# akashsengupta1997/STRAPS-3DHumanShapePose

Measured on AMD Instinct MI355X. Metric: bodies/sec, higher is better.
Workload: dtype fp32 (encoder convolutions as exact bf16x3 operand splits (six bf16 products per term); in-step SMPL blend contraction and skinning as 3-product fp16 splits (fp16x3_lbs: 22-bit operands); fp32 accumulate throughout)

## Files before the change

straps-3dhumanshapepose_amd/csrc/conv_wgrad.hip:

```cpp
#include "conv_wgrad_kernels.h"

namespace {

constexpr int F_TAP_F32 = STRAPS_WG_FAMILY_TAP_F32, F_HALO_F32 = STRAPS_WG_FAMILY_HALO_F32, F_TAP_X3 = STRAPS_WG_FAMILY_TAP_X3,
              F_HALO_X3 = STRAPS_WG_FAMILY_HALO_X3, F_TAP_X3F = STRAPS_WG_FAMILY_TAP_X3F;
constexpr int HALO_NG = 2;

inline int splits_for(int target, int tiles, long long max_s) {
    long long s = (target + tiles - 1) / tiles;
    if (s > max_s) s = max_s;
    return s < 1 ? 1 : (int)s;
}

bool halo_plan(int family, int cp, int batch, int h, int w, int cin, int cout, int kh, int kw, int stride, int pad, WgradPlan* pl) {
    if (!(kh == 3 && kw == 3 && stride == 1 && pad == 1)) return false;
    if (w < 8 || (w & (w - 1)) != 0) return false;
    const int cw = w < 32 ? w : 32, rpc = cp / cw;
    if (h % rpc != 0) return false;
    int lg = 0;
    while ((1 << lg) < cw) ++lg;
    WgradHaloGeom& g = pl->halo;
    g = {h, w, cin, cout, cw, lg, rpc, w / cw, h / rpc, batch * (h / rpc) * (w / cw), 0, cin / 64};
    const int tiles = (cout / 64) * (cin / 64);
    const int s = splits_for(WGRAD_CUS, tiles, (g.nchunks + 3) / 4);
    g.chunks_per_split = (g.nchunks + s - 1) / s;
    const int lds = family == F_HALO_F32 ? HALO_NG * 2 * W3PX * 64 * 4 : 2 * 3 * (cp + (cp == 32 ? 128 : 136)) * 64 * 2;
    pl->q = {family, 64, 64, cp, tiles, (g.nchunks + g.chunks_per_split - 1) / g.chunks_per_split, g.chunks_per_split, g.nchunks, 9, lds, 0};
    return true;
}

inline int tap_lds(int family, int bco, int bci) { return 2 * 32 * (bco + bci) * (family == F_TAP_F32 ? 4 : 3 * 2); }

void tap_plan(int family, int bco, int bci, int target, long long max_s, WgradPlan* pl) {
    WgradTapGeom& g = pl->tap;
    g.ct = g.Cout / bco; g.it = g.Cin / bci;
    const int taps = g.R * g.S, tiles = taps * g.ct * g.it, splits = splits_for(target, tiles, max_s);
    g.rows_per_split = (int)((((long long)g.M + splits - 1) / splits + 31) / 32 * 32);
    pl->q = {family, bco, bci, 0, tiles, splits, g.rows_per_split, g.M, taps, tap_lds(family, bco, bci), 0};
}

inline bool wgrad_big_tile(const WgradTapGeom& g) { return g.Cin % 128 == 0 && g.Cout % 128 == 0 && g.R * g.S == 1 && g.M >= 8192; }

void tap_f32_plan(WgradPlan* pl) {
    const bool big = wgrad_big_tile(pl->tap);
    tap_plan(F_TAP_F32, big ? 128 : 64, big ? 128 : 64, (big ? 2 : 6) * WGRAD_CUS, ((long long)pl->tap.M + 127) / 128, pl);
}

void tap_x3_block(const WgradTapGeom& g, int* bco, int* bci) {
    const int cin = g.Cin, cout = g.Cout;
    *bco = *bci = wgrad_big_tile(g) ? 128 : 64;
    if (g.R * g.S == 1) {
        if (g.M >= 32768 && cout % 256 == 0 && cin % 128 == 0) { *bco = 256; *bci = 128; }
        else if (g.M <= 8192 && cout % 128 == 0 && cin % 128 == 0) {
            if (g.stride == 1 && cout > cin) { *bco = 64; *bci = 128; }
            else { *bco = 128; *bci = 64; }
        }
    } else if (cout % 256 == 0 && cin % 128 == 0) { *bco = 256; *bci = 128; }
    else if (cout % 128 == 0 && cin % 64 == 0) { *bco = 128; *bci = 64; }
}

void tap_x3_plan(int bco, int bci, WgradPlan* pl) {
    const long long max_s = ((long long)pl->tap.M + 127) / 128;
    if (bco == bci) {
        tap_plan(F_TAP_X3, bco, bci, (bco == 128 ? 1 : 6) * WGRAD_CUS, max_s, pl);
        return;
    }
    WgradPlan f32 = *pl;
    tap_f32_plan(&f32);
    const int per_cu = (160 * 1024) / tap_lds(F_TAP_X3, bco, bci);
    tap_plan(F_TAP_X3, bco, bci, WGRAD_CUS * (per_cu < 1 ? 1 : per_cu), max_s < f32.q.splits ? max_s : f32.q.splits, pl);
}

void tap_x3f_block(int cin, int cout, int* bco, int* bci) {
    if (cout % 256 == 0 && cin == 64) { *bco = 256; *bci = 64; }
    else if (cin % 256 == 0 && cout == 64) { *bco = 64; *bci = 256; }
    else if (cout % 256 == 0 && cin % 128 == 0 && cout >= cin) { *bco = 256; *bci = 128; }
    else if (cin % 256 == 0 && cout % 128 == 0) { *bco = 128; *bci = 256; }
    else if (cout % 128 == 0 && cin % 128 == 0) { *bco = 128; *bci = 128; }
    else { *bco = 64; *bci = 64; }
}

inline bool reads_planes(const WgradPlan& pl) { return pl.q.family == F_TAP_X3 || pl.q.family == F_HALO_X3; }

}

int straps_internal_wgrad_plan(const char* who, int form, int batch, int h, int w, int cin, int cout, int kh, int kw, int stride, int pad, WgradPlan* pl) {
    *pl = WgradPlan{};
    const bool planes = form == STRAPS_WG_ROUTE_PLANES, x3f = form == STRAPS_WG_ROUTE_F32_1X1;
    STRAPS_REQUIRE(cin % 64 == 0 && cout % 64 == 0, "%s: need cin%%64==0 and cout%%64==0 (cin=%d cout=%d)", who, cin, cout);
    STRAPS_REQUIRE(!x3f || (kh == 1 && kw == 1 && pad == 0 && stride >= 1), "%s: 1x1 filters without padding only", who);
    WgradTapGeom& g = pl->tap;
    g = {batch, h, w, cin, cout, kh, kw, stride, pad, (h + 2 * pad - kh) / stride + 1, (w + 2 * pad - kw) / stride + 1};
    if (!x3f && halo_plan(planes ? F_HALO_X3 : F_HALO_F32, 32, batch, h, w, cin, cout, kh, kw, stride, pad, pl)) {
        WgradPlan p64 = *pl;
        if (planes && halo_plan(F_HALO_X3, 64, batch, h, w, cin, cout, kh, kw, stride, pad, &p64) && p64.q.splits <= pl->q.splits) *pl = p64;
    } else {
        const long long M = (long long)batch * g.Ho * g.Wo;
        STRAPS_REQUIRE(M < (1LL << 31) && (!x3f || M > 0), "%s: problem too large (or empty)", who);
        g.M = (int)M;
        int bco, bci;
        if (x3f) {
            tap_x3f_block(cin, cout, &bco, &bci);
            tap_plan(F_TAP_X3F, bco, bci, (bco == 64 && bci == 64 ? 2 : 1) * WGRAD_CUS, (M + 63) / 64, pl);
        } else if (planes && (kh * kw > 1 || (cin >= 128 && cout >= 128))) {
            tap_x3_block(g, &bco, &bci);
            tap_x3_plan(bco, bci, pl);
        } else {
            tap_f32_plan(pl);
        }
    }
#ifdef STRAPS_TOOLS
    if (pl->q.family == F_TAP_X3) {
        if (const int v = STRAPS_TOOL_ENV_INT("STRAPS_WGRAD_TILE", 0)) {
            const int o = v / 1000, i = v % 1000, sq = wgrad_big_tile(pl->tap) ? 128 : 64;
            const bool ok = (o == 64 || o == 128 || o == 256) && (i == 64 || i == 128 || i == 256) && !(o == 256 && i == 256) && cout % o == 0 && cin % i == 0 &&
                            !(o == 128 && i == 128 && sq != 128);
            tap_x3_plan(ok ? o : sq, ok ? i : sq, pl);
        }
    }
    static const int abl = STRAPS_TOOL_ENV_INT("STRAPS_WGRAD3_ABL", 0);
    if (pl->q.family == F_HALO_X3 && pl->q.chunk_px == 64) pl->abl = abl;
#endif
    pl->q.part_bytes = (int64_t)pl->q.splits * cout * pl->q.taps * cin * (int64_t)sizeof(float);
    return STRAPS_OK;
}

int straps_internal_wgrad_reduce(const float* part, float* dw_oihw, int splits, int cout, int cin, int taps, int accumulate, hipStream_t st) {
    const long long n = (long long)cout * taps * cin;
    hipLaunchKernelGGL(wgrad_reduce_kernel, dim3((unsigned)(n / 256)), dim3(256), 0, st, part, dw_oihw, splits, cout, cin, taps, accumulate);
    STRAPS_CHECK_LAUNCH("wgrad_reduce_kernel");
    return STRAPS_OK;
}

extern "C" int straps_conv_wgrad_plan(int route, int batch, int h, int w, int cin, int cout, int kh, int kw, int stride, int pad, straps_wgrad_plan_t* out) {
    STRAPS_REQUIRE(out && route >= STRAPS_WG_ROUTE_F32 && route <= STRAPS_WG_ROUTE_F32_1X1, "straps_conv_wgrad_plan: null pointer or unknown route %d", route);
    WgradPlan pl;
    const int rc = straps_internal_wgrad_plan("straps_conv_wgrad_plan", route, batch, h, w, cin, cout, kh, kw, stride, pad, &pl);
    if (rc == STRAPS_OK) *out = pl.q;
    return rc;
}

extern "C" size_t straps_conv_wgrad_workspace_bytes(int batch, int h, int w, int cin, int cout, int kh, int kw, int stride, int pad) {
    WgradPlan pl;
    const int rc = straps_internal_wgrad_plan("straps_conv_wgrad_workspace_bytes", STRAPS_WG_ROUTE_F32, batch, h, w, cin, cout, kh, kw, stride, pad, &pl);
    return rc == STRAPS_OK ? (size_t)pl.q.part_bytes : 0;
}

extern "C" int straps_conv_wgrad_x3_on_planes(int batch, int h, int w, int cin, int cout, int kh, int kw, int stride, int pad) {
    WgradPlan pl;
    return straps_internal_wgrad_plan("straps_conv_wgrad_x3_on_planes", STRAPS_WG_ROUTE_PLANES, batch, h, w, cin, cout, kh, kw, stride, pad, &pl) == STRAPS_OK && reads_planes(pl);
}

namespace {

constexpr int wkey(int family, int chunk_px, int bco, int bci) { return (family << 24) | (chunk_px << 18) | (bco << 9) | bci; }

int wgrad_launch(const WgradPlan& pl, const float* x, const float* dy, const u16* x3, long long xps, const u16* dy3, long long dps, float* dw_oihw,
                 void* workspace, int accumulate, void* stream) {
    const straps_wgrad_plan_t& q = pl.q;
    float* part = (float*)workspace;
    hipStream_t st = (hipStream_t)stream;
    const dim3 grid(q.tiles, q.splits);
    const size_t lds = (size_t)q.lds_bytes;
    WgradP tf{x, dy, part, pl.tap};
    Wgrad3P hf{x, dy, part, pl.halo};
    WgradXP tx{x3, dy3, xps, dps, part, pl.tap};
    Wgrad3XP hx{x3, dy3, xps, dps, part, pl.halo, (long long)pl.tap.B * pl.tap.H * pl.tap.W};
#define WGRAD_LAUNCH(KERN, THREADS, P)                                       \
    do {                                                                     \
        if (lds >= 64 * 1024) STRAPS_RAISE_LDS((KERN), lds, #KERN);          \
        hipLaunchKernelGGL((KERN), grid, dim3(THREADS), lds, st, P);         \
        STRAPS_CHECK_LAUNCH(#KERN);                                          \
    } while (0)
    switch (wkey(q.family, q.chunk_px, q.bco, q.bci)) {
    case wkey(F_TAP_F32, 0, 64, 64): WGRAD_LAUNCH((conv_wgrad_kernel<64, 64>), 256, tf); break;
    case wkey(F_TAP_F32, 0, 128, 128): WGRAD_LAUNCH((conv_wgrad_kernel<128, 128>), 256, tf); break;
    case wkey(F_HALO_F32, 32, 64, 64): WGRAD_LAUNCH((conv_wgrad3x3_kernel<HALO_NG>), 256 * HALO_NG, hf); break;
    case wkey(F_HALO_X3, 32, 64, 64): WGRAD_LAUNCH((conv_wgrad3x3_x3_kernel<HALO_NG, 32>), 256 * HALO_NG, hx); break;
    case wkey(F_HALO_X3, 64, 64, 64):
#ifdef STRAPS_TOOLS
        if (pl.abl) {
            auto kern = pl.abl == 1 ? conv_wgrad3x3_x3_kernel<HALO_NG, 64, 1> : pl.abl == 2 ? conv_wgrad3x3_x3_kernel<HALO_NG, 64, 2>
                      : pl.abl == 3 ? conv_wgrad3x3_x3_kernel<HALO_NG, 64, 3> : pl.abl == 4 ? conv_wgrad3x3_x3_kernel<HALO_NG, 64, 4> : conv_wgrad3x3_x3_kernel<HALO_NG, 64, 5>;
            (void)hipFuncSetAttribute((const void*)kern, hipFuncAttributeMaxDynamicSharedMemorySize, (int)lds);
            hipLaunchKernelGGL(kern, grid, dim3(256 * HALO_NG), lds, st, hx);
            STRAPS_CHECK_LAUNCH("conv_wgrad3x3_x3_kernel (ablation)");
            return STRAPS_OK;
        }
#endif
        WGRAD_LAUNCH((conv_wgrad3x3_x3_kernel<HALO_NG, 64>), 256 * HALO_NG, hx);
        break;
    case wkey(F_TAP_X3, 0, 64, 64): WGRAD_LAUNCH((conv_wgrad_x3_kernel<64, 64>), 256, tx); break;
    case wkey(F_TAP_X3, 0, 128, 128): WGRAD_LAUNCH((conv_wgrad_x3_kernel<128, 128>), 256, tx); break;
    case wkey(F_TAP_X3, 0, 256, 128): WGRAD_LAUNCH((conv_wgrad_x3_kernel<256, 128>), 256, tx); break;
    case wkey(F_TAP_X3, 0, 128, 64): WGRAD_LAUNCH((conv_wgrad_x3_kernel<128, 64>), 256, tx); break;
    case wkey(F_TAP_X3, 0, 64, 128): WGRAD_LAUNCH((conv_wgrad_x3_kernel<64, 128>), 256, tx); break;
#ifdef STRAPS_TOOLS
    case wkey(F_TAP_X3, 0, 256, 64): WGRAD_LAUNCH((conv_wgrad_x3_kernel<256, 64>), 256, tx); break;
    case wkey(F_TAP_X3, 0, 64, 256): WGRAD_LAUNCH((conv_wgrad_x3_kernel<64, 256>), 256, tx); break;
    case wkey(F_TAP_X3, 0, 128, 256): WGRAD_LAUNCH((conv_wgrad_x3_kernel<128, 256>), 256, tx); break;
#endif
    default: STRAPS_REQUIRE(false, "conv weight gradient: no kernel for family %d, block %d x %d", q.family, q.bco, q.bci);
    }
#undef WGRAD_LAUNCH
    return straps_internal_wgrad_reduce(part, dw_oihw, q.splits, pl.tap.Cout, pl.tap.Cin, q.taps, accumulate, st);
}

}

extern "C" int straps_conv_wgrad_x3(const float* x, const float* dy, const unsigned short* x3, long long x_plane_stride, const unsigned short* dy3,
                                    long long dy_plane_stride, float* dw_oihw, void* workspace, int batch, int h, int w, int cin, int cout, int kh,
                                    int kw, int stride, int pad, int accumulate, void* stream) {
    STRAPS_REQUIRE(dw_oihw && workspace, "straps_conv_wgrad_x3: null pointer");
    WgradPlan pl;
    const int rc = straps_internal_wgrad_plan("straps_conv_wgrad_x3", (x3 && dy3) ? STRAPS_WG_ROUTE_PLANES : STRAPS_WG_ROUTE_F32, batch, h, w, cin, cout, kh, kw, stride, pad, &pl);
    if (rc != STRAPS_OK) return rc;
    if (reads_planes(pl)) {
        STRAPS_REQUIRE(x_plane_stride % 8 == 0 && dy_plane_stride % 8 == 0, "straps_conv_wgrad_x3: plane strides must be multiples of 8 elements");
        const size_t adv = straps_conv_wgrad_workspace_bytes(batch, h, w, cin, cout, kh, kw, stride, pad);
        STRAPS_REQUIRE((size_t)pl.q.part_bytes <= adv, "straps_conv_wgrad_x3: the plan's partials (%lld bytes) exceed the advertised workspace (%zu)", (long long)pl.q.part_bytes, adv);
    } else {
        STRAPS_REQUIRE(x && dy, "straps_conv_wgrad_x3: this shape runs on the fp32 tensors, which are NULL (see straps_conv_wgrad_x3_on_planes)");
    }
    return wgrad_launch(pl, x, dy, x3, x_plane_stride, dy3, dy_plane_stride, dw_oihw, workspace, accumulate, stream);
}

extern "C" int straps_conv_wgrad(const float* x, const float* dy, float* dw_oihw, void* workspace, int batch, int h, int w, int cin,
                                 int cout, int kh, int kw, int stride, int pad, int accumulate, void* stream) {
    STRAPS_REQUIRE(x && dy && dw_oihw && workspace, "straps_conv_wgrad: null pointer");
    return straps_conv_wgrad_x3(x, dy, nullptr, 0, nullptr, 0, dw_oihw, workspace, batch, h, w, cin, cout, kh, kw, stride, pad, accumulate, stream);
}
```

straps-3dhumanshapepose_amd/csrc/conv_wgrad_kernels.h:

```cpp
#pragma once
#include "common.h"
#include "conv_wgrad_plan.h"

namespace {

struct WgradP {
    const float* x;
    const float* dy;
    float* part;
    WgradTapGeom g;
};

__device__ __attribute__((aligned(16))) float k_zero16w[4] = {0.f, 0.f, 0.f, 0.f};

template <int BCO, int BCI>
__global__ __launch_bounds__(256) void conv_wgrad_kernel(WgradP p) {
    constexpr int STG = 32 * (BCO + BCI);
    constexpr int LPD = BCO / 4, PWD = 64 / LPD, RDD = 8 / PWD;
    constexpr int LPX = BCI / 4, PWX = 64 / LPX, RDX = 8 / PWX;
    constexpr int MI = BCO / 64, NI = BCI / 64;
    extern __shared__ __attribute__((aligned(16))) float smem[];
    const int tid = threadIdx.x, lane = tid & 63, wave = tid >> 6;
    const int wave_u = __builtin_amdgcn_readfirstlane(wave);
    const int wm = wave >> 1, wn = wave & 1;
// ... 503 lines not shown
#pragma unroll
        for (int q = 0; q < DR; ++q) {
            if (NG > 1 && (q & 1) != grp) continue;
#pragma unroll
            for (int pl = 0; pl < 3; ++pl)
                __builtin_amdgcn_global_load_lds((const __attribute__((address_space(1))) void*)(dbase + d_off[q] + pl * p.dps),
                                                 (__attribute__((address_space(3))) void*)(D + (pl * DPX + 32 * q + 8 * wave_u) * 64), 16, 0, 0);
        }
#pragma unroll
        for (int q = 0; q < XR; ++q) {
            if (q * 32 + 8 * wave_u >= npatch || q * 32 + 8 * wave_u >= XPX) break;
            if (NG > 1 && ((q + DR) & 1) != grp) continue;
            const int hi = ho0 + x_pr[q], wi = wo0 + x_pc[q];
            const bool ok = (unsigned)hi < (unsigned)p.g.H && (unsigned)wi < (unsigned)p.g.W;
            const u16* src = ok ? xsrc + (x_pr[q] * p.g.W + x_pc[q]) * 32 + x_g[q] : zsrc;
            const long long ps = ok ? p.xps : 0;
#pragma unroll
            for (int pl = 0; pl < 3; ++pl)
                __builtin_amdgcn_global_load_lds((const __attribute__((address_space(1))) void*)(src + pl * ps),
                                                 (__attribute__((address_space(3))) void*)(X + (pl * XPX + 32 * q + 8 * wave_u) * 64), 16, 0, 0);
        }
    };

    const int t = lane & 15, ch16 = (lane >> 4) & 1, kh = lane >> 5;
    auto row_off = [&](int slot_px, int c4) {
        const int g = (c4 >> 3) ^ (((slot_px >> 1) & 1) << 2);
        return slot_px * 64 + g * 8 + (c4 & 4);
    };
    int d_fo[KSG][2], x_fo[KSG][2];
#pragma unroll
    for (int ks = 0; ks < KSG; ++ks)
#pragma unroll
        for (int r = 0; r < 2; ++r) {
            const int px = (grp + NG * ks) * 16 + kh * 8 + r * 4 + (t >> 2);
            d_fo[ks][r] = row_off(px, wm * 32 + ch16 * 16 + (t & 3) * 4);
            x_fo[ks][r] = (px >> p.g.cw_log2) * pw + (px & (p.g.cw - 1));
        }
    const int x_c4 = wn * 32 + ch16 * 16 + (t & 3) * 4;

    f32x16 acc[9];
#pragma unroll
    for (int tp = 0; tp < 9; ++tp)
#pragma unroll
        for (int q = 0; q < 16; ++q) acc[tp][q] = 0.f;
    if (cbeg < cend) dma_chunk(cbeg, 0);
    constexpr int TA[6] = {1, 0, 2, 0, 1, 0};
    constexpr int TB[6] = {1, 2, 0, 1, 0, 0};
    for (int c = cbeg; c < cend; ++c) {
        const int stage = (c - cbeg) & 1;
        asm volatile("s_waitcnt vmcnt(0)" ::: "memory");
        __builtin_amdgcn_s_barrier();
        asm volatile("" ::: "memory");
        if (c + 1 < cend && !(ABL & 1)) dma_chunk(c + 1, stage ^ 1);
        const u16* D = smem + ((ABL & 1) ? 0 : stage) * STAGE;
        const u16* X = D + 3 * DPX * 64;
        __builtin_amdgcn_s_setprio(1);
#pragma unroll
        for (int ks = 0; ks < KSG; ++ks) {
            bf16x8w a[3];
#pragma unroll
            for (int pl = 0; pl < 3; ++pl) a[pl] = tr_frag(D + pl * DPX * 64 + d_fo[ks][0], D + pl * DPX * 64 + d_fo[ks][1]);
#pragma unroll
            for (int tp0 = 0; tp0 < 9; tp0 += W3X_TG) {
                bf16x8w b[W3X_TG][3];
#pragma unroll
                for (int u = 0; u < W3X_TG; ++u) {
                    const int tp = tp0 + u;
                    if (tp >= 9) break;
                    const int sh = (ABL & 4) ? 0 : (tp / 3) * pw + (tp % 3);
                    const int o0 = row_off(x_fo[ks][0] + sh, x_c4), o1 = row_off(x_fo[ks][1] + sh, x_c4);
#pragma unroll
                    for (int pl = 0; pl < 3; ++pl) b[u][pl] = tr_frag(X + pl * XPX * 64 + o0, X + pl * XPX * 64 + o1);
                }
                if (ABL & 2) {
#pragma unroll
                    for (int u = 0; u < W3X_TG; ++u)
                        if (tp0 + u < 9)
#pragma unroll
                            for (int pl = 0; pl < 3; ++pl) acc[0][pl] += (float)b[u][pl][0] + (float)a[pl][1];
                    continue;
                }
#pragma unroll
                for (int e = 0; e < 6; ++e)
#pragma unroll
                    for (int u = 0; u < W3X_TG; ++u)
                        if (tp0 + u < 9) acc[tp0 + u] = __builtin_amdgcn_mfma_f32_32x32x16_bf16(a[TA[e]], b[u][TB[e]], acc[tp0 + u], 0, 0, 0);
            }
        }
        __builtin_amdgcn_s_setprio(0);
    }
    if constexpr (NG > 1) {
        float* R = smem_f + ((wave * 3) * 16) * 64 + lane;
#pragma unroll
        for (int rd = 0; rd < 3; ++rd) {
            __syncthreads();
            if (grp == 1) {
#pragma unroll
                for (int tp = 0; tp < 3; ++tp)
#pragma unroll
                    for (int q = 0; q < 16; ++q) R[(tp * 16 + q) * 64] = acc[rd * 3 + tp][q];
            }
            __syncthreads();
            if (grp == 0) {
#pragma unroll
                for (int tp = 0; tp < 3; ++tp)
#pragma unroll
                    for (int q = 0; q < 16; ++q) acc[rd * 3 + tp][q] += R[(tp * 16 + q) * 64];
            }
        }
        if (grp != 0) return;
    }
    const int i = lane & 31;
    float* o = p.part + (long long)blockIdx.y * p.g.Cout * 9 * p.g.Cin;
#pragma unroll
    for (int tp = 0; tp < 9; ++tp)
#pragma unroll
        for (int q = 0; q < 16; ++q) {
            const int co = co0 + wm * 32 + mfma_row(q, lane);
            o[((long long)co * 9 + tp) * p.g.Cin + ci0 + wn * 32 + i] = acc[tp][q];
        }
}

__global__ __launch_bounds__(256) void wgrad_reduce_kernel(const float* __restrict__ part, float* __restrict__ dw, int splits,
                                                           int Cout, int Cin, int RS, int accumulate) {
    __shared__ f32x4 red[4][64];
    const long long n = (long long)Cout * RS * Cin;
    const int lane = threadIdx.x & 63, sg = threadIdx.x >> 6;
    const long long idx = ((long long)blockIdx.x * 64 + lane) * 4;
    f32x4 s = {0.f, 0.f, 0.f, 0.f};
    int k = sg;
    for (; k + 12 < splits; k += 16) {
        const f32x4 v0 = *reinterpret_cast<const f32x4*>(part + (long long)k * n + idx);
        const f32x4 v1 = *reinterpret_cast<const f32x4*>(part + (long long)(k + 4) * n + idx);
        const f32x4 v2 = *reinterpret_cast<const f32x4*>(part + (long long)(k + 8) * n + idx);
        const f32x4 v3 = *reinterpret_cast<const f32x4*>(part + (long long)(k + 12) * n + idx);
        s += (v0 + v1) + (v2 + v3);
    }
    for (; k < splits; k += 4) s += *reinterpret_cast<const f32x4*>(part + (long long)k * n + idx);
    red[sg][lane] = s;
    __syncthreads();
    if (sg != 0) return;
    s = (red[0][lane] + red[1][lane]) + (red[2][lane] + red[3][lane]);
    const int ci = (int)(idx % Cin);
    long long t = idx / Cin;
    const int tap = (int)(t % RS);
    const int co = (int)(t / RS);
#pragma unroll
    for (int e = 0; e < 4; ++e) {
        const long long o = ((long long)co * Cin + ci + e) * RS + tap;
        dw[o] = accumulate ? dw[o] + s[e] : s[e];
    }
}

}
```

straps-3dhumanshapepose_amd/csrc/elementwise.hip:

```cpp
#include "common.h"

namespace {

__global__ __launch_bounds__(256) void pack_krsc_kernel(const float* __restrict__ src, float* __restrict__ dst, int O, int C, int R, int S) {
    const long long i = (long long)blockIdx.x * 256 + threadIdx.x;
    const long long n = (long long)O * C * R * S;
    if (i >= n) return;
    const int c = (int)(i % C);
    long long t = i / C;
    const int s = (int)(t % S); t /= S;
    const int r = (int)(t % R);
    const int o = (int)(t / R);
    dst[i] = src[(((long long)o * C + c) * R + r) * S + s];
}

__global__ __launch_bounds__(256) void pack_crsk_flip_kernel(const float* __restrict__ src, float* __restrict__ dst, int O, int C, int R, int S) {
    const long long i = (long long)blockIdx.x * 256 + threadIdx.x;
    const long long n = (long long)O * C * R * S;
    if (i >= n) return;
    const int o = (int)(i % O);
    long long t = i / O;
    const int s = (int)(t % S); t /= S;
    const int r = (int)(t % R);
    const int c = (int)(t / R);
    dst[i] = src[(((long long)o * C + c) * R + (R - 1 - r)) * S + (S - 1 - s)];
}

constexpr int PK_T = 32, PK_RS = 9, PK_LD = PK_T * PK_RS + 1;
__device__ __forceinline__ long long wk_index(int row, int tap, int k, int rows, int K) {
    return (((long long)tap * (K >> 5) + (k >> 5)) * rows + row) * 32 + (k & 31);
}
__global__ __launch_bounds__(256) void pack_batched_kernel(const straps_pack_desc_t* __restrict__ descs, int n, u16* __restrict__ k3_all,
                                                           u16* __restrict__ c3_all, long long ps) {
    __shared__ float tile[PK_T * PK_LD];
    const int tid = threadIdx.x;
    int d = 0;
    long long base = 0;
    for (long long u = blockIdx.x;; u += gridDim.x) {
        long long units = 0;
        int ot = 0, ct = 0, rt = 0;
        for (; d < n; ++d) {
            ot = (descs[d].o + PK_T - 1) / PK_T;
            ct = (descs[d].c + PK_T - 1) / PK_T;
            rt = (descs[d].r * descs[d].s + PK_RS - 1) / PK_RS;
            units = (long long)ot * ct * rt;
            if (u < base + units) break;
            base += units;
        }
        if (d >= n) return;
        const straps_pack_desc_t D = descs[d];
        const int RS = D.r * D.s;
        u16* const k3 = (D.c & 31) ? nullptr : k3_all;
        u16* const c3 = (D.o & 31) ? nullptr : c3_all;
        int v = (int)(u - base);
        const int ri = v % rt; v /= rt;
        const int ci = v % ct;
        const int oi = v / ct;
        const int o0 = oi * PK_T, c0 = ci * PK_T, rs0 = ri * PK_RS;
        const int no = min(PK_T, D.o - o0), nc = min(PK_T, D.c - c0), nr = min(PK_RS, RS - rs0);
        const int run = nc * nr;
        if (nr == PK_RS && RS == PK_RS && nc == PK_T && (D.c & 3) == 0 && (reinterpret_cast<uintptr_t>(D.src) & 15) == 0) {
            constexpr int RUN4 = PK_T * PK_RS / 4;
            for (int idx = tid; idx < no * RUN4; idx += 256) {
                const int o = idx / RUN4, q = idx - o * RUN4;
                const f32x4 v = *reinterpret_cast<const f32x4*>(D.src + ((long long)(o0 + o) * D.c + c0) * PK_RS + q * 4);
                float* t = tile + o * PK_LD + q * 4;
                t[0] = v[0]; t[1] = v[1]; t[2] = v[2]; t[3] = v[3];
            }
        } else {
            for (int idx = tid; idx < no * run; idx += 256) {
                const int o = idx / run, k = idx - o * run;
                const int c = k / nr, j = k - c * nr;
                tile[o * PK_LD + c * PK_RS + j] = D.src[((long long)(o0 + o) * D.c + c0 + c) * RS + rs0 + j];
            }
        }
        __syncthreads();
        const bool v4k = k3 && ((D.c | D.first) & 3) == 0, v4c = c3 && ((D.o | D.first) & 3) == 0;
        if (D.dst_krsc || (k3 && !v4k)) {
            for (int idx = tid; idx < no * nr * PK_T; idx += 256) {
                const int c = idx & (PK_T - 1);
                const int k = idx >> 5;
                const int j = k % nr, o = k / nr;
                if (c < nc) {
                    const long long at = ((long long)(o0 + o) * RS + rs0 + j) * D.c + c0 + c;
                    const float v = tile[o * PK_LD + c * PK_RS + j];
                    if (D.dst_krsc) D.dst_krsc[at] = v;
                    if (k3 && !v4k) {
                        u16 b1, b2, b3;
                        split3(v, b1, b2, b3);
                        const long long w = D.first + wk_index(o0 + o, rs0 + j, c0 + c, D.o, D.c);
                        k3[w] = b1; k3[ps + w] = b2; k3[2 * ps + w] = b3;
                    }
                }
            }
        }
        if (v4k) {
            for (int idx = tid; idx < no * nr * (PK_T / 4); idx += 256) {
                const int c = (idx & (PK_T / 4 - 1)) * 4;
                const int k = idx >> 3;
                const int o = nr == PK_RS ? k / PK_RS : k / nr, j = k - o * nr;
                if (c < nc) {
                    const float* t = tile + o * PK_LD + c * PK_RS + j;
                    const f32x4 v = {t[0], t[PK_RS], t[2 * PK_RS], t[3 * PK_RS]};
                    store_planes4(k3, ps, D.first + wk_index(o0 + o, rs0 + j, c0 + c, D.o, D.c), v);
                }
            }
        }
        if (D.dst_crsk || (c3 && !v4c)) {
            for (int idx = tid; idx < nc * nr * PK_T; idx += 256) {
                const int o = idx & (PK_T - 1);
                const int k = idx >> 5;
                const int j = k % nr, c = k / nr;
                if (o < no) {
                    const long long at = ((long long)(c0 + c) * RS + (RS - 1 - (rs0 + j))) * D.o + o0 + o;
                    const float v = tile[o * PK_LD + c * PK_RS + j];
                    if (D.dst_crsk) D.dst_crsk[at] = v;
                    if (c3 && !v4c) {
                        u16 b1, b2, b3;
                        split3(v, b1, b2, b3);
                        const long long w = D.first + wk_index(c0 + c, RS - 1 - (rs0 + j), o0 + o, D.c, D.o);
                        c3[w] = b1; c3[ps + w] = b2; c3[2 * ps + w] = b3;
                    }
                }
            }
        }
        if (v4c) {
            for (int idx = tid; idx < nc * nr * (PK_T / 4); idx += 256) {
                const int o = (idx & (PK_T / 4 - 1)) * 4;
                const int k = idx >> 3;
                const int c = nr == PK_RS ? k / PK_RS : k / nr, j = k - c * nr;
                if (o < no) {
                    const float* t = tile + o * PK_LD + c * PK_RS + j;
                    const f32x4 v = {t[0], t[PK_LD], t[2 * PK_LD], t[3 * PK_LD]};
                    store_planes4(c3, ps, D.first + wk_index(c0 + c, RS - 1 - (rs0 + j), o0 + o, D.c, D.o), v);
                }
            }
        }
        __syncthreads();
    }
}

__global__ void bn_fold_kernel(const float* __restrict__ g, const float* __restrict__ b, const float* __restrict__ mean,
                               const float* __restrict__ var, float eps, float* __restrict__ scale, float* __restrict__ shift, int C) {
    const int c = blockIdx.x * blockDim.x + threadIdx.x;
    if (c >= C) return;
    const float sc = g[c] / sqrtf(var[c] + eps);
    scale[c] = sc;
    shift[c] = fmaf(-mean[c], sc, b[c]);
}

__global__ __launch_bounds__(256) void maxpool_kernel(const float* __restrict__ x, float* __restrict__ y, int B, int H, int W, int C,
                                                      int Ho, int Wo) {
    const int C4 = C >> 2;
    const long long n = (long long)B * Ho * Wo * C4;
    for (long long i = (long long)blockIdx.x * 256 + threadIdx.x; i < n; i += (long long)gridDim.x * 256) {
        const int c4 = (int)(i % C4);
        long long t = i / C4;
        const int wo = (int)(t % Wo); t /= Wo;
        const int ho = (int)(t % Ho);
        const int b = (int)(t / Ho);
        f32x4 m = {-INFINITY, -INFINITY, -INFINITY, -INFINITY};
#pragma unroll
        for (int r = 0; r < 3; ++r) {
            const int hi = 2 * ho - 1 + r;
            if ((unsigned)hi >= (unsigned)H) continue;
#pragma unroll
            for (int s = 0; s < 3; ++s) {
                const int wi = 2 * wo - 1 + s;
                if ((unsigned)wi >= (unsigned)W) continue;
                const f32x4 v = *reinterpret_cast<const f32x4*>(x + (((long long)b * H + hi) * W + wi) * C + c4 * 4);
#pragma unroll
                for (int e = 0; e < 4; ++e)
                    if (v[e] > m[e] || v[e] != v[e]) m[e] = v[e];
            }
        }
        *reinterpret_cast<f32x4*>(y + i * 4) = m;
    }
}

__global__ __launch_bounds__(256) void gap_kernel(const float* __restrict__ x, float* __restrict__ y, int B, int HW, int C) {
    const long long i = (long long)blockIdx.x * 256 + threadIdx.x;
    if (i >= (long long)B * C) return;
    const int c = (int)(i % C);
    const long long b = i / C;
    const float* p = x + b * HW * C + c;
    float s = 0.f;
    for (int k = 0; k < HW; ++k) s += p[(long long)k * C];
    y[i] = s / (float)HW;
}

__global__ __launch_bounds__(256) void bn_stats_finalize_kernel(const float* __restrict__ part, int nblocks, int C, double count,
                                                               const float* __restrict__ gamma, const float* __restrict__ beta, float eps,
                                                               float momentum, float* __restrict__ rmean, float* __restrict__ rvar,
                                                               float* __restrict__ scale, float* __restrict__ shift,
                                                               float* __restrict__ smean, float* __restrict__ sinv) {
    int c;
    double s1, s2;
    if (bn_partials_sum4(part, nblocks, C, s1, s2, c)) {
        const double mean = s1 / count;
        double var = s2 / count - mean * mean;
        if (var < 0.0) var = 0.0;
        const float inv = (float)(1.0 / sqrt(var + (double)eps));
        const float sc = gamma[c] * inv;
        scale[c] = sc;
        shift[c] = fmaf(-(float)mean, sc, beta[c]);
        if (smean) smean[c] = (float)mean;
        if (sinv) sinv[c] = inv;
        if (rmean) {
            const double unbiased = count > 1.0 ? var * count / (count - 1.0) : var;
            rmean[c] = fmaf(momentum, (float)mean, (1.f - momentum) * rmean[c]);
            rvar[c] = fmaf(momentum, (float)unbiased, (1.f - momentum) * rvar[c]);
        }
    }
}

__global__ __launch_bounds__(256) void bn_apply_kernel(const float* __restrict__ x, const float* __restrict__ scale,
                                                       const float* __restrict__ shift, const float* __restrict__ res, int relu,
                                                       float* __restrict__ y, u16* __restrict__ planes, long long ps, long long n4, int C4,
                                                       unsigned* __restrict__ bits, int tiled) {
    const long long first = (long long)blockIdx.x * 256 + threadIdx.x, step = (long long)gridDim.x * 256;
    const long long rows = n4 / C4;
    auto body = [&](long long i, long long r, int c4, const f32x4& sc, const f32x4& sh) {
        f32x4 v = *reinterpret_cast<const f32x4*>(x + i * 4);
#pragma unroll
        for (int q = 0; q < 4; ++q) v[q] = fmaf(v[q], sc[q], sh[q]);
        if (res) v += *reinterpret_cast<const f32x4*>(res + i * 4);
        if (relu) { v[0] = fmaxf(v[0], 0.f); v[1] = fmaxf(v[1], 0.f); v[2] = fmaxf(v[2], 0.f); v[3] = fmaxf(v[3], 0.f); }
        if (y) *reinterpret_cast<f32x4*>(y + i * 4) = v;
        if (planes) store_planes4_cm(planes, ps, r, c4 * 4, rows, v);
        if (bits) {
            unsigned wd = ((v[0] > 0.f ? 1u : 0u) | (v[1] > 0.f ? 2u : 0u) | (v[2] > 0.f ? 4u : 0u) | (v[3] > 0.f ? 8u : 0u)) << ((c4 & 7) * 4);
            wd |= __shfl_xor(wd, 1, 64);
            wd |= __shfl_xor(wd, 2, 64);
            wd |= __shfl_xor(wd, 4, 64);
            if ((c4 & 7) == 0) bits[r * (C4 >> 3) + (c4 >> 3)] = wd;
        }
    };
    if (tiled) {
        const int l = threadIdx.x & 63, w = threadIdx.x >> 6, wcg = tiled, ncb = (C4 >> 4) / wcg, trows = 16 / wcg;
        const int c4 = ((int)(blockIdx.x % ncb) * wcg + w % wcg) * 16 + (l >> 5) * 8 + (l & 7);
        const f32x4 sc = *reinterpret_cast<const f32x4*>(scale + c4 * 4);
        const f32x4 sh = *reinterpret_cast<const f32x4*>(shift + c4 * 4);
        const long long rstep = (long long)(gridDim.x / ncb) * trows;
        for (long long r = (long long)(blockIdx.x / ncb) * trows + (w / wcg) * 4 + ((l >> 3) & 3); r < rows; r += rstep) body(r * C4 + c4, r, c4, sc, sh);
    } else if (step % C4 == 0) {
        const int c4 = (int)(first % C4);
        const f32x4 sc = *reinterpret_cast<const f32x4*>(scale + c4 * 4);
        const f32x4 sh = *reinterpret_cast<const f32x4*>(shift + c4 * 4);
        const long long rstep = step / C4;
        long long r = first / C4;
        for (long long i = first; i < n4; i += step, r += rstep) body(i, r, c4, sc, sh);
    } else {
        for (long long i = first; i < n4; i += step) {
            const int c4 = (int)(i % C4);
            body(i, i / C4, c4, *reinterpret_cast<const f32x4*>(scale + c4 * 4), *reinterpret_cast<const f32x4*>(shift + c4 * 4));
        }
    }
}

__global__ void bn_fold_stats_kernel(const float* __restrict__ g, const float* __restrict__ b, const float* __restrict__ mean,
                                     const float* __restrict__ var, float eps, float* __restrict__ scale, float* __restrict__ shift,
                                     float* __restrict__ smean, float* __restrict__ sinv, int C) {
    const int c = blockIdx.x * blockDim.x + threadIdx.x;
    if (c >= C) return;
    const float inv = 1.0f / sqrtf(var[c] + eps);
    const float sc = g[c] / sqrtf(var[c] + eps);
    scale[c] = sc;
    shift[c] = fmaf(-mean[c], sc, b[c]);
    smean[c] = mean[c];
    sinv[c] = inv;
}

inline unsigned capped_grid(long long n) {
    long long g = (n + 255) / 256;
    return (unsigned)(g > 256 * 16 ? 256 * 16 : (g < 1 ? 1 : g));
}

}

extern "C" int straps_pack_conv_weight(const float* w_oihw, float* w_krsc, int cout, int cin, int kh, int kw, void* stream) {
    STRAPS_REQUIRE(w_oihw && w_krsc && cout > 0 && cin > 0 && kh > 0 && kw > 0, "straps_pack_conv_weight: bad arguments");
    const long long n = (long long)cout * cin * kh * kw;
    hipLaunchKernelGGL(pack_krsc_kernel, dim3((unsigned)((n + 255) / 256)), dim3(256), 0, (hipStream_t)stream, w_oihw, w_krsc, cout, cin, kh, kw);
    STRAPS_CHECK_LAUNCH("pack_krsc_kernel");
    return STRAPS_OK;
}

extern "C" int straps_pack_conv_weight_dgrad(const float* w_oihw, float* w_crsk, int cout, int cin, int kh, int kw, void* stream) {
    STRAPS_REQUIRE(w_oihw && w_crsk && cout > 0 && cin > 0 && kh > 0 && kw > 0, "straps_pack_conv_weight_dgrad: bad arguments");
    const long long n = (long long)cout * cin * kh * kw;
    hipLaunchKernelGGL(pack_crsk_flip_kernel, dim3((unsigned)((n + 255) / 256)), dim3(256), 0, (hipStream_t)stream, w_oihw, w_crsk, cout, cin, kh, kw);
    STRAPS_CHECK_LAUNCH("pack_crsk_flip_kernel");
    return STRAPS_OK;
}

extern "C" int straps_pack_conv_weights_batched(const straps_pack_desc_t* descs, int n, long long total, void* stream) {
    STRAPS_REQUIRE(descs && n > 0 && total > 0, "straps_pack_conv_weights_batched: bad arguments");
    long long blocks = (total + PK_T * PK_T * PK_RS - 1) / (PK_T * PK_T * PK_RS);
    if (blocks > 8192) blocks = 8192;
    hipLaunchKernelGGL(pack_batched_kernel, dim3((unsigned)blocks), dim3(256), 0, (hipStream_t)stream, descs, n, (u16*)nullptr, (u16*)nullptr, 0LL);
    STRAPS_CHECK_LAUNCH("pack_batched_kernel");
    return STRAPS_OK;
}

extern "C" int straps_pack_conv_weights_batched_x3(const straps_pack_desc_t* descs, int n, long long total, unsigned short* krsc_planes,
                                                   unsigned short* crsk_planes, long long plane_stride, void* stream) {
    STRAPS_REQUIRE(descs && n > 0 && total > 0, "straps_pack_conv_weights_batched_x3: bad arguments");
    STRAPS_REQUIRE(krsc_planes || crsk_planes, "straps_pack_conv_weights_batched_x3: no planes given (use straps_pack_conv_weights_batched)");
    STRAPS_REQUIRE(plane_stride >= total && plane_stride % 8 == 0, "straps_pack_conv_weights_batched_x3: plane_stride must be >= total and a multiple of 8");
    STRAPS_REQUIRE((reinterpret_cast<uintptr_t>(krsc_planes) & 15) == 0 && (reinterpret_cast<uintptr_t>(crsk_planes) & 15) == 0,
                   "straps_pack_conv_weights_batched_x3: plane buffers must be 16-byte aligned");
    long long blocks = (total + PK_T * PK_T * PK_RS - 1) / (PK_T * PK_T * PK_RS);
    if (blocks > 8192) blocks = 8192;
    hipLaunchKernelGGL(pack_batched_kernel, dim3((unsigned)blocks), dim3(256), 0, (hipStream_t)stream, descs, n, krsc_planes, crsk_planes, plane_stride);
    STRAPS_CHECK_LAUNCH("pack_batched_kernel");
    return STRAPS_OK;
}

extern "C" int straps_bn_fold(const float* gamma, const float* beta, const float* mean, const float* var, float eps, float* scale,
                              float* shift, int c, void* stream) {
    STRAPS_REQUIRE(gamma && beta && mean && var && scale && shift && c > 0, "straps_bn_fold: bad arguments");
    hipLaunchKernelGGL(bn_fold_kernel, dim3((c + 255) / 256), dim3(256), 0, (hipStream_t)stream, gamma, beta, mean, var, eps, scale, shift, c);
    STRAPS_CHECK_LAUNCH("bn_fold_kernel");
    return STRAPS_OK;
}

extern "C" int straps_bn_fold_stats(const float* gamma, const float* beta, const float* mean, const float* var, float eps, float* scale,
                                    float* shift, float* save_mean, float* save_invstd, int c, void* stream) {
    STRAPS_REQUIRE(gamma && beta && mean && var && scale && shift && save_mean && save_invstd && c > 0, "straps_bn_fold_stats: bad arguments");
    hipLaunchKernelGGL(bn_fold_stats_kernel, dim3((c + 255) / 256), dim3(256), 0, (hipStream_t)stream, gamma, beta, mean, var, eps, scale, shift, save_mean,
                       save_invstd, c);
    STRAPS_CHECK_LAUNCH("bn_fold_stats_kernel");
    return STRAPS_OK;
}

extern "C" int straps_maxpool_fwd(const float* x, float* y, int batch, int h, int w, int c, void* stream) {
    STRAPS_REQUIRE(x && y && batch > 0 && h > 0 && w > 0 && c > 0 && (c & 3) == 0, "straps_maxpool_fwd: bad arguments (c%%4 must be 0)");
    const int Ho = (h + 2 - 3) / 2 + 1, Wo = (w + 2 - 3) / 2 + 1;
    const long long n = (long long)batch * Ho * Wo * (c >> 2);
    hipLaunchKernelGGL(maxpool_kernel, dim3(capped_grid(n)), dim3(256), 0, (hipStream_t)stream, x, y, batch, h, w, c, Ho, Wo);
    STRAPS_CHECK_LAUNCH("maxpool_kernel");
    return STRAPS_OK;
}

extern "C" int straps_gap_fwd(const float* x, float* y, int batch, int hw, int c, void* stream) {
    STRAPS_REQUIRE(x && y && batch > 0 && hw > 0 && c > 0, "straps_gap_fwd: bad arguments");
    const long long n = (long long)batch * c;
    hipLaunchKernelGGL(gap_kernel, dim3((unsigned)((n + 255) / 256)), dim3(256), 0, (hipStream_t)stream, x, y, batch, hw, c);
    STRAPS_CHECK_LAUNCH("gap_kernel");
    return STRAPS_OK;
}

extern "C" int straps_bn_stats_finalize(const float* stats_partial, int nblocks, int c, long long count, const float* gamma,
                                        const float* beta, float eps, float momentum, float* running_mean, float* running_var,
                                        float* scale, float* shift, float* save_mean, float* save_invstd, void* stream) {
    STRAPS_REQUIRE(stats_partial && gamma && beta && scale && shift && nblocks > 0 && c > 0 && count > 0, "straps_bn_stats_finalize: bad arguments");
    STRAPS_REQUIRE((running_mean == nullptr) == (running_var == nullptr), "straps_bn_stats_finalize: running stats must be given together");
    hipLaunchKernelGGL(bn_stats_finalize_kernel, dim3((c + 3) / 4), dim3(256), 0, (hipStream_t)stream, stats_partial, nblocks, c, (double)count, gamma, beta,
                       eps, momentum, running_mean, running_var, scale, shift, save_mean, save_invstd);
    STRAPS_CHECK_LAUNCH("bn_stats_finalize_kernel");
    return STRAPS_OK;
}

extern "C" int straps_bn_apply(const float* x, const float* scale, const float* shift, const float* residual, int relu, float* y,
                               long long rows, int c, void* stream) {
    STRAPS_REQUIRE(x && scale && shift && y && rows > 0 && c > 0 && (c & 3) == 0, "straps_bn_apply: bad arguments (c%%4 must be 0)");
    const long long n4 = rows * (c >> 2);
    hipLaunchKernelGGL(bn_apply_kernel, dim3(capped_grid(n4)), dim3(256), 0, (hipStream_t)stream, x, scale, shift, residual, relu, y, (u16*)nullptr, 0LL, n4, c >> 2, (unsigned*)nullptr, 0);
    STRAPS_CHECK_LAUNCH("bn_apply_kernel");
    return STRAPS_OK;
}

static int bn_apply_x3_impl(const char* who, const float* x, const float* scale, const float* shift, const float* residual, int relu, float* y,
                            unsigned short* y_planes, long long plane_stride, unsigned* relu_bits, long long rows, int c, void* stream) {
    STRAPS_REQUIRE(x && scale && shift && (y_planes || y) && rows > 0 && c > 0 && (c & 31) == 0, "%s: bad arguments (c%%32 must be 0: chunk-major planes; c=%d)", who, c);
    STRAPS_REQUIRE(!y_planes || (plane_stride >= rows * c && plane_stride % 8 == 0), "%s: plane_stride must be >= rows*c and a multiple of 8", who);
    const long long n4 = rows * (c >> 2);
    const int tiled = straps_bn_tiled(rows, c >> 2);
    hipLaunchKernelGGL(bn_apply_kernel, dim3(tiled ? straps_bn_tiled_grid(rows, c >> 2, tiled) : straps_grid256_rows(n4, c >> 2)), dim3(256), 0, (hipStream_t)stream, x, scale, shift,
                       residual, relu, y, y_planes, plane_stride, n4, c >> 2, relu_bits, tiled);
    STRAPS_CHECK_LAUNCH("bn_apply_kernel");
    return STRAPS_OK;
}

extern "C" int straps_bn_apply_x3(const float* x, const float* scale, const float* shift, const float* residual, int relu, float* y,
                                  unsigned short* y_planes, long long plane_stride, long long rows, int c, void* stream) {
    return bn_apply_x3_impl("straps_bn_apply_x3", x, scale, shift, residual, relu, y, y_planes, plane_stride, nullptr, rows, c, stream);
}

extern "C" int straps_bn_apply_bits_x3(const float* x, const float* scale, const float* shift, const float* residual, float* y,
                                       unsigned short* y_planes, long long plane_stride, unsigned* relu_bits, long long rows, int c, void* stream) {
    STRAPS_REQUIRE(relu_bits, "straps_bn_apply_bits_x3: null bit buffer");
    return bn_apply_x3_impl("straps_bn_apply_bits_x3", x, scale, shift, residual, 1, y, y_planes, plane_stride, relu_bits, rows, c, stream);
}
```

Measured before the change: 8092.

## Add 3x3 wgrad reduce kernel, pipeline weight packing, and split GAP across waves

Adds a dedicated 3x3 weight-gradient split-reduce kernel. Each block handles one output channel and a 64-wide input slice, reduces the partials with vector loads, and transposes through LDS so the OIHW writes are coalesced instead of strided by 9. The batched weight-pack kernel now finds each unit's descriptor with a wave-wide prefix scan and ballot instead of a serial walk, and it prefetches the next unit's source into registers while the current one is emitted. Global average pooling now splits the spatial loop across four waves per 64 channels and combines the partial sums through LDS, which adds two barriers per 64-pixel chunk in return for more memory parallelism.

```diff
diff --git a/straps-3dhumanshapepose_amd/csrc/conv_wgrad.hip b/straps-3dhumanshapepose_amd/csrc/conv_wgrad.hip
--- a/straps-3dhumanshapepose_amd/csrc/conv_wgrad.hip
+++ b/straps-3dhumanshapepose_amd/csrc/conv_wgrad.hip
@@ -127,6 +127,11 @@
 
 int straps_internal_wgrad_reduce(const float* part, float* dw_oihw, int splits, int cout, int cin, int taps, int accumulate, hipStream_t st) {
     const long long n = (long long)cout * taps * cin;
+    if (taps == 9 && splits <= 28) {
+        hipLaunchKernelGGL(wgrad_reduce3x3_kernel, dim3((unsigned)(cout * (cin / 64))), dim3(WR3_THREADS), 0, st, part, dw_oihw, splits, cout, cin, accumulate);
+        STRAPS_CHECK_LAUNCH("wgrad_reduce3x3_kernel");
+        return STRAPS_OK;
+    }
     hipLaunchKernelGGL(wgrad_reduce_kernel, dim3((unsigned)(n / 256)), dim3(256), 0, st, part, dw_oihw, splits, cout, cin, taps, accumulate);
     STRAPS_CHECK_LAUNCH("wgrad_reduce_kernel");
     return STRAPS_OK;
diff --git a/straps-3dhumanshapepose_amd/csrc/conv_wgrad_kernels.h b/straps-3dhumanshapepose_amd/csrc/conv_wgrad_kernels.h
--- a/straps-3dhumanshapepose_amd/csrc/conv_wgrad_kernels.h
+++ b/straps-3dhumanshapepose_amd/csrc/conv_wgrad_kernels.h
@@ -679,4 +679,53 @@
     }
 }
 
+constexpr int WR3_THREADS = 4 * 9 * 16;
+__global__ __launch_bounds__(WR3_THREADS) void wgrad_reduce3x3_kernel(const float* __restrict__ part, float* __restrict__ dw, int splits,
+                                                                      int Cout, int Cin, int accumulate) {
+    __shared__ f32x4 red[4][144];
+    __shared__ float tr[64 * 9];
+    const long long n = (long long)Cout * 9 * Cin;
+    const int cb = Cin >> 6;
+    const int co = blockIdx.x / cb, ci0 = (blockIdx.x - co * cb) * 64;
+    const int sg = threadIdx.x / 144, item = threadIdx.x - sg * 144, tap = item >> 4, c4 = item & 15;
+    const float* const p = part + ((long long)co * 9 + tap) * Cin + ci0 + c4 * 4;
+    const f32x4 zero = {0.f, 0.f, 0.f, 0.f};
+    f32x4 s = zero;
+    int k = sg;
+    for (; k + 12 < splits; k += 16) {
+        const bool last = k + 28 >= splits;
+        f32x4 v[4], tl[3];
+#pragma unroll
+        for (int e = 0; e < 4; ++e) v[e] = *reinterpret_cast<const f32x4*>(p + (long long)(k + 4 * e) * n);
+#pragma unroll
+        for (int e = 0; e < 3; ++e) tl[e] = last && k + 16 + 4 * e < splits ? *reinterpret_cast<const f32x4*>(p + (long long)(k + 16 + 4 * e) * n) : zero;
+        s += (v[0] + v[1]) + (v[2] + v[3]);
+        if (last) {
+#pragma unroll
+            for (int e = 0; e < 3; ++e)
+                if (k + 16 + 4 * e < splits) s += tl[e];
+            k = splits;
+        }
+    }
+    {
+        f32x4 tl[3];
+#pragma unroll
+        for (int e = 0; e < 3; ++e) tl[e] = k + 4 * e < splits ? *reinterpret_cast<const f32x4*>(p + (long long)(k + 4 * e) * n) : zero;
+#pragma unroll
+        for (int e = 0; e < 3; ++e)
+            if (k + 4 * e < splits) s += tl[e];
+    }
+    red[sg][item] = s;
+    __syncthreads();
+    if (sg == 0) {
+        s = (red[0][item] + red[1][item]) + (red[2][item] + red[3][item]);
+#pragma unroll
+        for (int e = 0; e < 4; ++e) tr[(c4 * 4 + e) * 9 + tap] = s[e];
+    }
+    __syncthreads();
+    const long long o = ((long long)co * Cin + ci0) * 9 + threadIdx.x;
+    const float t = tr[threadIdx.x];
+    dw[o] = accumulate ? dw[o] + t : t;
 }
+
+}
diff --git a/straps-3dhumanshapepose_amd/csrc/elementwise.hip b/straps-3dhumanshapepose_amd/csrc/elementwise.hip
--- a/straps-3dhumanshapepose_amd/csrc/elementwise.hip
+++ b/straps-3dhumanshapepose_amd/csrc/elementwise.hip
@@ -30,51 +30,101 @@
 __device__ __forceinline__ long long wk_index(int row, int tap, int k, int rows, int K) {
     return (((long long)tap * (K >> 5) + (k >> 5)) * rows + row) * 32 + (k & 31);
 }
+struct PkUnit {
+    straps_pack_desc_t D;
+    int RS, o0, c0, rs0, no, nc, nr;
+    bool fast;
+};
+constexpr int PK_PRE = PK_T * PK_T * PK_RS / 256;
+__device__ __forceinline__ long long pk_readlane(long long v, int l) {
+    const unsigned lo = (unsigned)__builtin_amdgcn_readlane((int)(v & 0xffffffffll), l), hi = (unsigned)__builtin_amdgcn_readlane((int)(v >> 32), l);
+    return (long long)(((unsigned long long)hi << 32) | lo);
+}
 __global__ __launch_bounds__(256) void pack_batched_kernel(const straps_pack_desc_t* __restrict__ descs, int n, u16* __restrict__ k3_all,
                                                            u16* __restrict__ c3_all, long long ps) {
     __shared__ float tile[PK_T * PK_LD];
-    const int tid = threadIdx.x;
-    int d = 0;
-    long long base = 0;
-    for (long long u = blockIdx.x;; u += gridDim.x) {
-        long long units = 0;
-        int ot = 0, ct = 0, rt = 0;
-        for (; d < n; ++d) {
-            ot = (descs[d].o + PK_T - 1) / PK_T;
-            ct = (descs[d].c + PK_T - 1) / PK_T;
-            rt = (descs[d].r * descs[d].s + PK_RS - 1) / PK_RS;
-            units = (long long)ot * ct * rt;
-            if (u < base + units) break;
-            base += units;
-        }
-        if (d >= n) return;
-        const straps_pack_desc_t D = descs[d];
-        const int RS = D.r * D.s;
-        u16* const k3 = (D.c & 31) ? nullptr : k3_all;
-        u16* const c3 = (D.o & 31) ? nullptr : c3_all;
+    const int tid = threadIdx.x, lane = tid & 63;
+    int d0 = 0, lct = 0, lrt = 0;
+    long long cbase = 0, un = 0, inc = 0;
+    auto load_chunk = [&]() {
+        const int d = d0 + lane;
+        un = 0; lct = lrt = 0;
+        if (d < n) {
+            const int o = descs[d].o, c = descs[d].c, r = descs[d].r, s = descs[d].s;
+            lct = (c + PK_T - 1) / PK_T;
+            lrt = (r * s + PK_RS - 1) / PK_RS;
+            un = (long long)((o + PK_T - 1) / PK_T) * lct * lrt;
+        }
+        inc = un;
+#pragma unroll
+        for (int off = 1; off < 64; off <<= 1) {
+            const long long t = __shfl_up(inc, off, 64);
+            if (lane >= off) inc += t;
+        }
+    };
+    auto find = [&](long long u, PkUnit& U) -> bool {
+        int l;
+        for (;;) {
+            const unsigned long long hit = __ballot(u < cbase + inc);
+            if (hit) { l = __ffsll((long long)hit) - 1; break; }
+            cbase += pk_readlane(inc, 63);
+            d0 += 64;
+            if (d0 >= n) return false;
+            load_chunk();
+        }
+        const long long base = cbase + pk_readlane(inc - un, l);
+        const int ct = __builtin_amdgcn_readlane(lct, l), rt = __builtin_amdgcn_readlane(lrt, l);
+        U.D = descs[d0 + l];
+        const straps_pack_desc_t& D = U.D;
+        U.RS = D.r * D.s;
         int v = (int)(u - base);
         const int ri = v % rt; v /= rt;
         const int ci = v % ct;
         const int oi = v / ct;
-        const int o0 = oi * PK_T, c0 = ci * PK_T, rs0 = ri * PK_RS;
-        const int no = min(PK_T, D.o - o0), nc = min(PK_T, D.c - c0), nr = min(PK_RS, RS - rs0);
-        const int run = nc * nr;
-        if (nr == PK_RS && RS == PK_RS && nc == PK_T && (D.c & 3) == 0 && (reinterpret_cast<uintptr_t>(D.src) & 15) == 0) {
-            constexpr int RUN4 = PK_T * PK_RS / 4;
-            for (int idx = tid; idx < no * RUN4; idx += 256) {
+        U.o0 = oi * PK_T; U.c0 = ci * PK_T; U.rs0 = ri * PK_RS;
+        U.no = min(PK_T, D.o - U.o0); U.nc = min(PK_T, D.c - U.c0); U.nr = min(PK_RS, U.RS - U.rs0);
+        U.fast = U.nr == PK_RS && U.RS == PK_RS && U.nc == PK_T && (D.c & 3) == 0 && (reinterpret_cast<uintptr_t>(D.src) & 15) == 0;
+        return true;
+    };
+    constexpr int RUN4 = PK_T * PK_RS / 4;
+    auto fetch = [&](const PkUnit& U, f32x4 (&pre)[PK_PRE / 4]) {
+        if (!U.fast) return;
+        const straps_pack_desc_t& D = U.D;
+#pragma unroll
+        for (int i = 0; i < PK_PRE / 4; ++i) {
+            const int idx = tid + 256 * i;
+            if (idx < U.no * RUN4) {
                 const int o = idx / RUN4, q = idx - o * RUN4;
-                const f32x4 v = *reinterpret_cast<const f32x4*>(D.src + ((long long)(o0 + o) * D.c + c0) * PK_RS + q * 4);
-                float* t = tile + o * PK_LD + q * 4;
-                t[0] = v[0]; t[1] = v[1]; t[2] = v[2]; t[3] = v[3];
+                pre[i] = *reinterpret_cast<const f32x4*>(D.src + ((long long)(U.o0 + o) * D.c + U.c0) * PK_RS + q * 4);
+            }
+        }
+    };
+    auto stage = [&](const PkUnit& U, const f32x4 (&pre)[PK_PRE / 4]) {
+        if (U.fast) {
+#pragma unroll
+            for (int i = 0; i < PK_PRE / 4; ++i) {
+                const int idx = tid + 256 * i;
+                if (idx < U.no * RUN4) {
+                    const int o = idx / RUN4, q = idx - o * RUN4;
+                    float* t = tile + o * PK_LD + q * 4;
+                    t[0] = pre[i][0]; t[1] = pre[i][1]; t[2] = pre[i][2]; t[3] = pre[i][3];
+                }
             }
         } else {
-            for (int idx = tid; idx < no * run; idx += 256) {
+            const straps_pack_desc_t& D = U.D;
+            const int run = U.nc * U.nr;
+            for (int idx = tid; idx < U.no * run; idx += 256) {
                 const int o = idx / run, k = idx - o * run;
-                const int c = k / nr, j = k - c * nr;
-                tile[o * PK_LD + c * PK_RS + j] = D.src[((long long)(o0 + o) * D.c + c0 + c) * RS + rs0 + j];
-            }
-        }
-        __syncthreads();
+                const int c = k / U.nr, j = k - c * U.nr;
+                tile[o * PK_LD + c * PK_RS + j] = D.src[((long long)(U.o0 + o) * D.c + U.c0 + c) * U.RS + U.rs0 + j];
+            }
+        }
+    };
+    auto emit = [&](const PkUnit& U) {
+        const straps_pack_desc_t& D = U.D;
+        const int RS = U.RS, o0 = U.o0, c0 = U.c0, rs0 = U.rs0, no = U.no, nc = U.nc, nr = U.nr;
+        u16* const k3 = (D.c & 31) ? nullptr : k3_all;
+        u16* const c3 = (D.o & 31) ? nullptr : c3_all;
         const bool v4k = k3 && ((D.c | D.first) & 3) == 0, v4c = c3 && ((D.o | D.first) & 3) == 0;
         if (D.dst_krsc || (k3 && !v4k)) {
             for (int idx = tid; idx < no * nr * PK_T; idx += 256) {
@@ -98,7 +148,7 @@
             for (int idx = tid; idx < no * nr * (PK_T / 4); idx += 256) {
                 const int c = (idx & (PK_T / 4 - 1)) * 4;
                 const int k = idx >> 3;
-                const int o = nr == PK_RS ? k / PK_RS : k / nr, j = k - o * nr;
+                const int j = no == PK_T ? k / PK_T : k / no, o = k - j * no;
                 if (c < nc) {
                     const float* t = tile + o * PK_LD + c * PK_RS + j;
                     const f32x4 v = {t[0], t[PK_RS], t[2 * PK_RS], t[3 * PK_RS]};
@@ -128,7 +178,7 @@
             for (int idx = tid; idx < nc * nr * (PK_T / 4); idx += 256) {
                 const int o = (idx & (PK_T / 4 - 1)) * 4;
                 const int k = idx >> 3;
-                const int c = nr == PK_RS ? k / PK_RS : k / nr, j = k - c * nr;
+                const int j = nc == PK_T ? k / PK_T : k / nc, c = k - j * nc;
                 if (o < no) {
                     const float* t = tile + o * PK_LD + c * PK_RS + j;
                     const f32x4 v = {t[0], t[PK_LD], t[2 * PK_LD], t[3 * PK_LD]};
@@ -136,7 +186,27 @@
                 }
             }
         }
+    };
+    long long u = blockIdx.x;
+    auto next_unit = [&]() {
+        const long long v = u;
+        u += gridDim.x;
+        return v;
+    };
+    PkUnit cur, nxt;
+    f32x4 pre[PK_PRE / 4];
+    load_chunk();
+    if (!find(next_unit(), cur)) return;
+    fetch(cur, pre);
+    for (;;) {
+        stage(cur, pre);
         __syncthreads();
+        const bool more = find(next_unit(), nxt);
+        if (more) fetch(nxt, pre);
+        emit(cur);
+        if (!more) return;
+        __syncthreads();
+        cur = nxt;
     }
 }
 
@@ -179,14 +249,35 @@
 }
 
 __global__ __launch_bounds__(256) void gap_kernel(const float* __restrict__ x, float* __restrict__ y, int B, int HW, int C) {
-    const long long i = (long long)blockIdx.x * 256 + threadIdx.x;
-    if (i >= (long long)B * C) return;
-    const int c = (int)(i % C);
-    const long long b = i / C;
+    __shared__ float tile[64][64];
+    const int cl = threadIdx.x & 63, h = threadIdx.x >> 6;
+    const long long i = (long long)blockIdx.x * 64 + cl;
+    const bool live = i < (long long)B * C;
+    const int c = live ? (int)(i % C) : 0;
+    const long long b = live ? i / C : 0;
     const float* p = x + b * HW * C + c;
     float s = 0.f;
-    for (int k = 0; k < HW; ++k) s += p[(long long)k * C];
-    y[i] = s / (float)HW;
+    for (int k0 = 0; k0 < HW; k0 += 64) {
+        float v[16];
+#pragma unroll
+        for (int q = 0; q < 16; ++q) {
+            const int k = k0 + h + 4 * q;
+            v[q] = live && k < HW ? p[(long long)k * C] : 0.f;
+        }
+#pragma unroll
+        for (int q = 0; q < 16; ++q) tile[h + 4 * q][cl] = v[q];
+        __syncthreads();
+        if (h == 0) {
+            float r[64];
+#pragma unroll
+            for (int k = 0; k < 64; ++k) r[k] = tile[k][cl];
+#pragma unroll
+            for (int k = 0; k < 64; ++k)
+                if (k0 + k < HW) s += r[k];
+        }
+        __syncthreads();
+    }
+    if (h == 0 && live) y[i] = s / (float)HW;
 }
 
 __global__ __launch_bounds__(256) void bn_stats_finalize_kernel(const float* __restrict__ part, int nblocks, int C, double count,
@@ -271,6 +362,11 @@
     sinv[c] = inv;
 }
 
+inline long long pack_blocks(long long total) {
+    const long long blocks = (total + PK_T * PK_T * PK_RS - 1) / (PK_T * PK_T * PK_RS);
+    return blocks > 8192 ? 8192 : blocks;
+}
+
 inline unsigned capped_grid(long long n) {
     long long g = (n + 255) / 256;
     return (unsigned)(g > 256 * 16 ? 256 * 16 : (g < 1 ? 1 : g));
@@ -296,8 +392,7 @@
 
 extern "C" int straps_pack_conv_weights_batched(const straps_pack_desc_t* descs, int n, long long total, void* stream) {
     STRAPS_REQUIRE(descs && n > 0 && total > 0, "straps_pack_conv_weights_batched: bad arguments");
-    long long blocks = (total + PK_T * PK_T * PK_RS - 1) / (PK_T * PK_T * PK_RS);
-    if (blocks > 8192) blocks = 8192;
+    const long long blocks = pack_blocks(total);
     hipLaunchKernelGGL(pack_batched_kernel, dim3((unsigned)blocks), dim3(256), 0, (hipStream_t)stream, descs, n, (u16*)nullptr, (u16*)nullptr, 0LL);
     STRAPS_CHECK_LAUNCH("pack_batched_kernel");
     return STRAPS_OK;
@@ -310,8 +405,7 @@
     STRAPS_REQUIRE(plane_stride >= total && plane_stride % 8 == 0, "straps_pack_conv_weights_batched_x3: plane_stride must be >= total and a multiple of 8");
     STRAPS_REQUIRE((reinterpret_cast<uintptr_t>(krsc_planes) & 15) == 0 && (reinterpret_cast<uintptr_t>(crsk_planes) & 15) == 0,
                    "straps_pack_conv_weights_batched_x3: plane buffers must be 16-byte aligned");
-    long long blocks = (total + PK_T * PK_T * PK_RS - 1) / (PK_T * PK_T * PK_RS);
-    if (blocks > 8192) blocks = 8192;
+    const long long blocks = pack_blocks(total);
     hipLaunchKernelGGL(pack_batched_kernel, dim3((unsigned)blocks), dim3(256), 0, (hipStream_t)stream, descs, n, krsc_planes, crsk_planes, plane_stride);
     STRAPS_CHECK_LAUNCH("pack_batched_kernel");
     return STRAPS_OK;
@@ -346,7 +440,7 @@
 extern "C" int straps_gap_fwd(const float* x, float* y, int batch, int hw, int c, void* stream) {
     STRAPS_REQUIRE(x && y && batch > 0 && hw > 0 && c > 0, "straps_gap_fwd: bad arguments");
     const long long n = (long long)batch * c;
-    hipLaunchKernelGGL(gap_kernel, dim3((unsigned)((n + 255) / 256)), dim3(256), 0, (hipStream_t)stream, x, y, batch, hw, c);
+    hipLaunchKernelGGL(gap_kernel, dim3((unsigned)((n + 63) / 64)), dim3(256), 0, (hipStream_t)stream, x, y, batch, hw, c);
     STRAPS_CHECK_LAUNCH("gap_kernel");
     return STRAPS_OK;
 }
```

New measurement: 8140, median of 6. No clear change (+0.6%).
